# stulacy/bmm-mcmc

Measured on AMD Instinct MI355X. Metric: gibbs_sweeps_per_s, higher is better.
Workload: dtype f64; 1 GPU; c5: gibbs_collapsed K=20 N=10000000 P=100, 1 chain per GPU; sampler=collapsed, K=20, N=10000000, P=100, batch=2500000, chains=1, chains_per_gpu=1, burn_sweeps=30, x_layout=bit planes, ceil(P/32) words per observation, packed once at hand-over

## Files before the change

### bmm-mcmc_amd/csrc/chain.hip

```cpp
#include <hip/hip_runtime.h>
#include <hip/hip_ext.h>
#include <rccl/rccl.h>

#include <dlfcn.h>
#include <emmintrin.h>
#include <sched.h>
#include <sys/mman.h>

#include <cmath>
#include <cstdarg>
#include <cstdio>
#include <cstdint>
#include <cstdlib>
#include <cstring>
#include <atomic>
#include <chrono>
#include <condition_variable>
#include <exception>
#include <functional>
#include <limits>
#include <memory>
#include <mutex>
#include <new>
#include <string>
// ... 778 lines not shown
    if (old) HIP_TRY(hipStreamSynchronize(old));
    int rc = chain_stream_create(c, true);
    if (rc) { c->stream = old; c->stream_kind = old_kind; return rc; }
    chain_stream_release(c->device, old, old_kind);
    return BMM_OK;
}

struct Carver {
    char* base;
    size_t used = 0;
    template <class T> T* take(size_t n) {
        const size_t off = (used + 255) & ~(size_t)255;
        used = off + n * sizeof(T);
        return base ? reinterpret_cast<T*>(base + off) : nullptr;
    }
};

int chain_alloc(bmm_chain* c) {
    const ChainParams& p = c->p;
    HIP_TRY(hipSetDevice(c->device));
    {
        int rcs = chain_stream_create(c, false);
        if (rcs) return rcs;
    }
    const size_t nz = (size_t)p.N;
    const size_t ns = (size_t)p.K * p.P, nn = (size_t)p.K;
    const size_t ntab = (size_t)layout_of(c).doubles() + (explicit_params(p.mode) ? 0 : 2 * (size_t)pk_tq_doubles(layout_of(c)));
    auto carve = [&](Carver& a) {
        c->dNk = a.take<int32_t>(nn);
        c->dDNk = a.take<int32_t>(nn * kDeltaReps);
        c->dS = a.take<int32_t>(ns);
        c->dDS = a.take<int32_t>(ns * kDeltaReps);
        c->dTab = a.take<double>(ntab);
#ifdef BMM_DIAG
        c->dDiag = a.take<unsigned long long>(16);
#endif
        c->dSelfDone = a.take<int>(1);
        c->dViable = a.take<int>(1);
        c->dDNkAlt = a.take<int32_t>(nn * kDeltaReps);
        c->dDSAlt = a.take<int32_t>(ns * kDeltaReps);
#ifdef BMM_DEBUG_HOOKS
        c->dDbgFlag = a.take<int>(1);
        c->dPkStat = a.take<unsigned long long>(3);
#endif
        const size_t zeroed = a.used;
        c->dAlpha = a.take<double>(1);
        c->dPi = a.take<double>(nn);
        c->dTheta = a.take<double>(ns);
        c->dZ[0] = a.take<int32_t>(nz);
        c->dZ[1] = a.take<int32_t>(nz);
        return zeroed;
    };
    Carver measure{nullptr};
    carve(measure);
    c->arena = static_cast<char*>(dev_pool().get(c->device, measure.used, &c->arena_bytes));
    if (!c->arena) return set_err(BMM_E_HIP, "allocating the chain's state failed: %s", hipGetErrorString(hipGetLastError()));
    Carver real{c->arena};
    const size_t zeroed = carve(real);
    if (c->generic) HIP_TRY(hipMalloc(&c->dScratch, (size_t)c->scratch_stride * p.Kc * sizeof(double)));
    HIP_TRY(hipMemsetAsync(c->arena, 0, zeroed, c->stream));
    HIP_TRY(hipMemsetAsync(c->dZ[0], 0xff, nz * sizeof(int32_t), c->stream));
    HIP_TRY(hipMemcpyAsync(c->dAlpha, &c->alpha0, sizeof(double), hipMemcpyHostToDevice, c->stream));
    HIP_TRY(hipStreamSynchronize(c->stream));
    return BMM_OK;
}

int dbg_labels_ok(bmm_chain* c) {
#ifdef BMM_DEBUG_HOOKS
    int flag = 0;
    HIP_TRY(hipMemcpy(&flag, c->dDbgFlag, sizeof(int), hipMemcpyDeviceToHost));
    if (flag) return set_err(BMM_E_STATE, "a resample kernel produced or read a label outside [0, K): kernel bug (debug-hooks build check)");
#else
    (void)c;
#endif
    return BMM_OK;
}

int launch_resample(bmm_chain* c, const int32_t* z_in, int32_t* z_out, int64_t lo, int64_t hi,
                    uint32_t sweep) {
    ResampleArgs a{};
    a.X = c->dX; a.Xb = c->dXb; a.z_in = z_in; a.z_out = z_out; a.tab = c->dTab; a.dNk = c->dDNk; a.dS = c->dDS;
    a.lo = lo; a.hi = hi; a.sweep = sweep; a.minus_in_lds = c->minus_in_lds; a.diag = c->dDiag;
    a.dbg_flag = c->dDbgFlag; a.dbg_inject = (dbg_env("BMM_DEBUG_BADLABEL") ? 1 : 0) | (dbg_env("BMM_DEBUG_STRAGGLER") ? 2 : 0) |
                                             (dbg_env("BMM_DEBUG_DRAW_FALLBACK") ? 4 : 0) | (dbg_env("BMM_DEBUG_DRAW_NOEPS") ? 8 : 0);
    a.Nk = c->dNk; a.S = c->dS; a.alpha_ptr = c->dAlpha; a.self_done = c->dSelfDone;
#ifdef BMM_DEBUG_HOOKS
    a.pk_stat = c->dPkStat;
    a.pk_defer_every = c->pk_defer_every;
#endif
    const bool emit = c->probs_dst != nullptr;
    const bool use_generic = c->generic || (emit && !c->fn_emit);
    const bool self_launch = c->form.self && !emit && !use_generic;
    if (self_launch) { a.dNk_prev = c->dDNk; a.dS_prev = c->dDS; a.dNk = c->dDNkAlt; a.dS = c->dDSAlt; }
    const KernelForm& form = emit ? c->form_emit : c->form;
    const int gmax = emit ? c->grid_max_emit : c->grid_max;
    const int64_t ntiles = use_generic ? 1 : (hi - lo + tile_of(form) - 1) / tile_of(form);
    int grid = (int)(ntiles < gmax ? ntiles : gmax);
    if (use_generic) {
        const int64_t nt256 = (hi - lo + 255) / 256;
        const int64_t maxb = c->scratch_stride / 256;
        grid = (int)(nt256 < maxb ? nt256 : maxb);
    }
    if (emit) { a.wts = c->dWts; a.wtot = c->dWtot; }
    hipEvent_t e0 = nullptr, e1 = nullptr;
    if (c->prof > 0 && sweep % (uint32_t)c->prof == 0) {
        if (c->ev_used + 2 > c->ev.size()) {
            hipEvent_t a0, a1;
            HIP_TRY(hipEventCreate(&a0));
            HIP_TRY(hipEventCreate(&a1));
            c->ev.push_back(a0); c->ev.push_back(a1);
        }
        e0 = c->ev[c->ev_used]; e1 = c->ev[c->ev_used + 1];
        c->ev_used += 2;
    }
    if (use_generic) {
        if (e0) hipExtLaunchKernelGGL(k_resample_generic, dim3(grid), dim3(256), 0, c->stream, e0, e1, 0, c->p, a,
                                      c->dScratch, c->scratch_stride);
        else hipLaunchKernelGGL(k_resample_generic, dim3(grid), dim3(256), 0, c->stream, c->p, a, c->dScratch,
                                c->scratch_stride);
    } else {
        const resample_fn fn = emit ? c->fn_emit : c->fn;
        const int nt = form.nt;
        const size_t lds = emit ? c->lds_bytes_base : c->lds_bytes;
        if (e0) hipExtLaunchKernelGGL(fn, dim3(grid), dim3(nt), (uint32_t)lds, c->stream, e0, e1, 0, c->p, a);
        else hipLaunchKernelGGL(fn, dim3(grid), dim3(nt), lds, c->stream, c->p, a);
    }
    HIP_TRY(hipGetLastError());
    if (self_launch) { std::swap(c->dDNk, c->dDNkAlt); std::swap(c->dDS, c->dDSAlt); }
    if (emit) {
        const int64_t nb = (hi - lo + 255) / 256;
        hipLaunchKernelGGL(k_probs_finish, dim3((unsigned)(nb < 4096 ? nb : 4096)), dim3(256), 0, c->stream, c->p,
                           c->dTab, c->dWts, c->dWtot, z_in, lo, hi, c->probs_dst);
        HIP_TRY(hipGetLastError());
    }
    return BMM_OK;
}

int probs_alloc(bmm_chain* c, bool with_matrix) {
    const size_t n = (size_t)c->p.N;
    if (c->bits && !c->generic && !c->fn_emit) {
        const resample_fn fn = lookup(c->form_emit);
        int pe = 0;
        const hipError_t e = kernel_fits(fn, c->form_emit.nt, c->lds_bytes_base, &pe);
        if (e != hipSuccess) return set_err(BMM_E_HIP, "kernel set-up failed: %s", hipGetErrorString(e));
        c->fn_emit = fn;
        c->grid_max_emit = (pe < 1 ? 1 : pe) * c->num_cus;
    }
    if (!c->dWts) HIP_TRY(hipMalloc(&c->dWts, n * c->p.Kc * sizeof(double)));
    if (!c->dWtot) HIP_TRY(hipMalloc(&c->dWtot, n * sizeof(double)));
    if (with_matrix && !c->dProbs) HIP_TRY(hipMalloc(&c->dProbs, n * c->p.K * sizeof(double)));
    if (!c->fn_emit && !c->dScratch) {
        c->scratch_stride = generic_threads(c->p.Kc);
        HIP_TRY(hipMalloc(&c->dScratch, (size_t)c->scratch_stride * c->p.Kc * sizeof(double)));
    }
    return BMM_OK;
}

int launch_reduce_deltas(bmm_chain* c) {
    const int n = c->p.K * c->p.P + c->p.K;
    hipLaunchKernelGGL(k_reduce_deltas, dim3((n + 255) / 256), dim3(256), 0, c->stream, c->p, c->dDNk, c->dDS);
    HIP_TRY(hipGetLastError());
    return BMM_OK;
}

int launch_count_tables(bmm_chain* c) {
    if (c->alloc_on)
        hipLaunchKernelGGL(k_alloc_tables, dim3(c->p.KT), dim3(kCountTablesThreads), 0, c->stream, c->p, c->dNk, c->dS,
                           c->dDNk, c->dDS, (const int32_t*)c->dEaK, c->alloc_a, c->dTab);
    else if (c->temper_on)
        hipLaunchKernelGGL(k_temper_tables, dim3(c->p.KT), dim3(kCountTablesThreads), 0, c->stream, c->p, c->dNk, c->dS,
                           c->dDNk, c->dDS, (const double*)c->dAlpha, c->temper_b, c->dTab);
    else if (c->fs_mask)
        hipLaunchKernelGGL(k_count_tables<true>, dim3(c->p.KT), dim3(kCountTablesThreads), 0, c->stream, c->p, c->dNk, c->dS,
                           c->dDNk, c->dDS, c->dAlpha, c->dTab, (const uint32_t*)c->dFsMask, 0);
    else
        hipLaunchKernelGGL(k_count_tables<false>, dim3(c->p.KT), dim3(kCountTablesThreads), 0, c->stream, c->p, c->dNk, c->dS,
                           c->dDNk, c->dDS, c->dAlpha, c->dTab, (const uint32_t*)nullptr, c->form.pk && !c->generic ? 1 : 0);
    HIP_TRY(hipGetLastError());
    return BMM_OK;
}

int launch_score(bmm_chain* c, ScoreArgs a, bool loo) {
    const ChainParams& p = c->p;
    a.tab = c->dTab;
    if (!explicit_params(p.mode)) {
        double* const tab = loo ? c->dLooTab : c->dPredTab;
// ... 4344 lines not shown
                if (d == ch->slot) return set_err(BMM_E_ARG, "one chain per device here; chains on one device share (bmm_chain_share_data)");
            if (ch->p.N != chains[0]->p.N || ch->p.P != chains[0]->p.P) return set_err(BMM_E_ARG, "the chains differ in N or P");
            devs.push_back(ch->slot);
            int rc = bmm_chain_planes(ch, &bufs[(size_t)c], &words);
            if (rc) return rc;
        }
        int rc = rccl_broadcast_words(devs, bufs, (size_t)words);
        for (int c = 1; c < n_chains && rc == BMM_OK; ++c) rc = bmm_chain_planes_filled(chains[c]);
        return rc;
    });
}

int bmm_multi_selfcheck(int n_devices, const int* devices, int64_t words) {
    return guarded([&]() -> int {
        if (n_devices < 1 || !devices || words < 1) return set_err(BMM_E_ARG, "bad argument");
        std::vector<int> devs(devices, devices + n_devices);
        for (int q = 0; q < n_devices; ++q)
            for (int r2 = 0; r2 < q; ++r2)
                if (devs[(size_t)q] == devs[(size_t)r2]) return set_err(BMM_E_ARG, "devices must be distinct");
        std::vector<uint32_t> pat((size_t)words), got((size_t)words);
        for (int64_t i = 0; i < words; ++i) pat[(size_t)i] = (uint32_t)i * 2654435761u + 12345u;
        std::vector<DevBuf> bufs((size_t)n_devices);
        std::vector<void*> ptrs((size_t)n_devices);
        for (int q = 0; q < n_devices; ++q) {
            HIP_TRY(hipSetDevice(devs[(size_t)q]));
            HIP_TRY(bufs[(size_t)q].alloc((size_t)words * 4));
            ptrs[(size_t)q] = bufs[(size_t)q].p;
            if (q == 0) HIP_TRY(hipMemcpy(ptrs[0], pat.data(), (size_t)words * 4, hipMemcpyHostToDevice));
            else HIP_TRY(hipMemset(ptrs[(size_t)q], 0, (size_t)words * 4));
        }
        if (n_devices == 1) {
            Rccl r;
            int rc = rccl_open(r);
            if (rc) return rc;
            ncclComm_t comm = nullptr;
            ncclResult_t e = r.CommInitAll(&comm, 1, devs.data());
            if (e != ncclSuccess) return set_err(BMM_E_RCCL, "ncclCommInitAll failed: %s", r.GetErrorString(e));
            hipStream_t st = nullptr;
            hipError_t he = hipStreamCreateWithFlags(&st, hipStreamNonBlocking);
            if (he == hipSuccess) {
                e = r.Broadcast(ptrs[0], ptrs[0], (size_t)words, ncclUint32, 0, comm, st);
                he = hipStreamSynchronize(st);
                (void)hipStreamDestroy(st);
            }
            (void)r.CommDestroy(comm);
            if (he != hipSuccess) return set_err(BMM_E_HIP, "self-check stream failed: %s", hipGetErrorString(he));
            if (e != ncclSuccess) return set_err(BMM_E_RCCL, "ncclBroadcast failed: %s", r.GetErrorString(e));
        } else {
            int rc = rccl_broadcast_words(devs, ptrs, (size_t)words);
            if (rc) return rc;
        }
        for (int q = 0; q < n_devices; ++q) {
            HIP_TRY(hipSetDevice(devs[(size_t)q]));
            HIP_TRY(hipMemcpy(got.data(), ptrs[(size_t)q], (size_t)words * 4, hipMemcpyDeviceToHost));
            if (std::memcmp(got.data(), pat.data(), (size_t)words * 4) != 0)
                return set_err(BMM_E_RCCL, "device %d holds different words after the broadcast", devs[(size_t)q]);
        }
        return BMM_OK;
    });
}

int bmm_device_math(int device, int op, const double* in, const double* in2, double* out, int64_t n) {
    if (!in || !out || n < 0 || op < 0 || op > 5) return set_err(BMM_E_ARG, "bad argument");
    if (op == 2 && !in2) return set_err(BMM_E_ARG, "division needs in2");
    HIP_TRY(hipSetDevice(device));
    DevBuf bi, bi2, bo;
    HIP_TRY(bi.alloc(n * sizeof(double)));
    HIP_TRY(bo.alloc(n * sizeof(double)));
    HIP_TRY(hipMemcpy(bi.p, in, n * sizeof(double), hipMemcpyHostToDevice));
    if (in2) {
        HIP_TRY(bi2.alloc(n * sizeof(double)));
        HIP_TRY(hipMemcpy(bi2.p, in2, n * sizeof(double), hipMemcpyHostToDevice));
    }
    if (op == 5)
        hipLaunchKernelGGL(k_test_lgamma, dim3((unsigned)((n + 255) / 256)), dim3(256), 0, 0, bi.as<double>(), bo.as<double>(), n);
    else
        hipLaunchKernelGGL(k_test_math, dim3((unsigned)((n + 255) / 256)), dim3(256), 0, 0, op, bi.as<double>(),
                           bi2.as<double>(), bo.as<double>(), n);
    HIP_TRY(hipGetLastError());
    HIP_TRY(hipMemcpy(out, bo.p, n * sizeof(double), hipMemcpyDeviceToHost));
    return BMM_OK;
}

int bmm_device_variates(int device, int kind, double p, double q, uint64_t seed, uint32_t sweep, double* out,
                        int64_t n) {
    if (!out || n < 0 || kind < 0 || kind > 2) return set_err(BMM_E_ARG, "bad argument");
    HIP_TRY(hipSetDevice(device));
    DevBuf bo;
    HIP_TRY(bo.alloc(n * sizeof(double)));
    hipLaunchKernelGGL(k_test_variates, dim3((unsigned)((n + 255) / 256)), dim3(256), 0, 0, kind, p, q, seed, sweep,
                       bo.as<double>(), n);
    HIP_TRY(hipGetLastError());
    HIP_TRY(hipMemcpy(out, bo.p, n * sizeof(double), hipMemcpyDeviceToHost));
    return BMM_OK;
}

}
```

### bmm-mcmc_amd/csrc/kernels.hip.h

```cpp
#pragma once
#include <hip/hip_runtime.h>
#include <stdint.h>

#include "bmm_spec.h"

namespace bmm {

typedef __attribute__((address_space(3))) double lds_f64;

constexpr int kMaxP = 128;
constexpr int lcm_(int a, int b) { int x = a; while (x % b) x += a; return x; }
constexpr int kChunkP = kMaxP / lcm_(lcm_(kGroupW, kGroupWAlt), kGroupWm) * lcm_(lcm_(kGroupW, kGroupWAlt), kGroupWm);
constexpr int kMaxCats = 64;
constexpr int kMaxCatsAny = 1024;

enum : int { MODE_COLLAPSED = 0, MODE_DP = 1, MODE_SB = 2, MODE_FULL = 3 };
__host__ __device__ inline bool explicit_params(int mode) { return mode == MODE_SB || mode == MODE_FULL; }

struct TableLayout {
    int G, KT, Gm, M;
    __host__ __device__ int tp() const { return 0; }
    __host__ __device__ int cp() const { return G * KT * M; }
    __host__ __device__ int cm() const { return cp() + KT; }
    __host__ __device__ int nk() const { return cm() + KT; }
// ... 1044 lines not shown
typedef float pk_f2 __attribute__((ext_vector_type(2)));
typedef __attribute__((address_space(3))) pk_f2 lds_pk_f2;
typedef __attribute__((address_space(3))) float lds_f32;
constexpr int kOwnPadMax = ((kMaxP + kGroupWm - 1) / kGroupWm + kOwnSub - 1) / kOwnSub * kOwnSub;
static_assert(kOwnPadMax <= 64, "pk_exact_count loads the own-cluster entries one per lane");

__device__ __forceinline__ int pk_dp_label(const int32_t* NkT, int K, int Kused, int new_label, int zo, int zoc) {
    const int own_single = (zo >= 0 && NkT[zoc] == 1) ? 1 : 0;
    if (Kused - own_single < K - 1) {
        int zn = new_label;
        if (own_single && (zn < 0 || zo < zn)) zn = zo;
        return zn;
    }
    int best = -1, bs = 0;
    for (int k = 0; k < K; ++k) {
        const int sz = NkT[k] - (k == zo ? 1 : 0);
        if (sz > 0 && (best < 0 || sz < bs)) { best = k; bs = sz; }
    }
    return best >= 0 ? best : zoc;
}
__device__ __forceinline__ unsigned pk_field(int bit, unsigned mask, uint32_t b0, uint32_t b1, uint32_t b2, uint32_t b3) {
    const int wd = bit >> 5;
    return __builtin_amdgcn_alignbit(word_of(wd + 1, b0, b1, b2, b3), word_of(wd, b0, b1, b2, b3), (unsigned)(bit & 31)) & mask;
}

__device__ __forceinline__ double pk_bcast(double x, int j) {
    const long long b = __double_as_longlong(x);
    const uint64_t e = (uint64_t)(uint32_t)__builtin_amdgcn_readlane((int)(uint32_t)b, j) |
                       ((uint64_t)(uint32_t)__builtin_amdgcn_readlane((int)(uint32_t)(b >> 32), j) << 32);
    return __longlong_as_double((long long)e);
}

template <int KT, int GW>
__device__ __forceinline__ int pk_exact_count(const ChainParams& p, const ResampleArgs& a, const TableLayout& L,
                                              uint32_t w0, uint32_t w1, uint32_t w2, uint32_t w3, int zo, double u,
                                              const lds_f64* ET, int lane) {
    constexpr int GM = 1 << GW;
    constexpr int GR = KT <= 4 ? 6 : KT <= 8 ? 10 : 20;
    static_assert((kMaxP + GW - 1) / GW <= 64, "lane g holds the field of group g");
    const int G = p.G;
    const int zoc = zo < 0 ? 0 : zo;
    const int k = lane < KT ? lane : KT - 1;
    const double* const tp = a.tab + L.tp();
    const int gmp = L.gm_pad();
    const int go = lane < gmp ? lane : gmp - 1;
    const double oe = a.tab[L.tm() + ((size_t)go * KT + zoc) * kGroupMm + pk_field(go * kGroupWm, kGroupMm - 1, w0, w1, w2, w3)];
    const unsigned koff = (unsigned)k * GM;
    const int gl = lane < G ? lane : G - 1;
    const int fld = (int)pk_field(gl * GW, GM - 1, w0, w1, w2, w3);
    double sc = 0.0;
#pragma unroll 1
    for (int g0 = 0; g0 < G; g0 += GR) {
        double tv[GR];
#pragma unroll
        for (int v = 0; v < GR; ++v) {
            const int g = g0 + v < G ? g0 + v : G - 1;
            const double* const row = tp + ((size_t)g * KT * GM + (unsigned)__builtin_amdgcn_readlane(fld, g));
            tv[v] = row[koff];
        }
#pragma unroll
        for (int v = 0; v < GR; ++v)
            if (g0 + v < G) sc = sc + tv[v];
    }
    double own = 0.0;
#pragma unroll 1
    for (int g = 0; g < gmp; ++g) own = own + pk_bcast(oe, g);
    if (k == zo) sc = own;
    double m = neg_inf();
#pragma unroll
    for (int j = 0; j < KT; ++j) m = max_score(m, pk_bcast(sc, j));
    const double w = expw_tab(sc - m, ET);
    double run = 0.0, cdf = 0.0;
#pragma unroll
    for (int j = 0; j < KT; ++j) {
        run = run + pk_bcast(w, j);
        cdf = lane == j ? run : cdf;
    }
    const double t = u * run;
    int zn = (int)__popcll(__ballot(lane < KT && t >= cdf));
    if (!(m > neg_inf())) zn = zoc;
    return zn;
}

template <int KT, int NT, int GW>
__global__ __launch_bounds__(NT) void k_resample_pk(ChainParams p, ResampleArgs a) {
    static_assert(KT % 2 == 0 && KT <= 32, "pairs of categories, one lane per category in pk_exact_count");
    constexpr int GM = 1 << GW;
    constexpr int KP = KT / 2;
    constexpr int CH = KP <= 12 ? KP : KP / 2;
    static_assert(KP % CH == 0, "chunking");
    constexpr int NW = NT / 64;
    extern __shared__ __attribute__((aligned(16))) char smem[];
    const TableLayout L{p.G, KT, p.Gm, GM};
    double* const lds = reinterpret_cast<double*>(smem);
    const int nq_d = pk_tq_doubles(L), tail_d = L.tm() - L.nk();
    const volatile lds_pk_f2* const Tq = (const volatile lds_pk_f2*)lds;
    const volatile lds_f32* const Tm32 = (const volatile lds_f32*)(lds + nq_d);
    double* const tail = lds + 2 * nq_d;
    const int32_t* const NkT = reinterpret_cast<const int32_t*>(tail);
    const lds_f64* const ET = (const lds_f64*)(tail + (L.et() - L.nk()));
    int32_t* const hist = reinterpret_cast<int32_t*>(tail + tail_d);
    const int P = p.P, G = p.G, K = p.K;
    const int tid = threadIdx.x, lane = tid & 63;
    int* const next_chunk = hist + K * P + K;
    DIAG(const unsigned long long d_entry = diag_stamp();)
    const int64_t nchunks = (a.hi - a.lo + 63) / 64;
    const int64_t cpw = (nchunks + gridDim.x - 1) / gridDim.x;
    const int64_t wg_c0 = (int64_t)blockIdx.x * cpw;
    const int64_t wg_cn = nchunks - wg_c0 < cpw ? nchunks - wg_c0 : cpw;
    const int W = (P + 31) / 32;
    const int wave = __builtin_amdgcn_readfirstlane(tid >> 6);
    int64_t tile = wg_c0 + wave;
    const bool has_tile = wave < wg_cn;
    TilePos pos = tile_pos(a, has_tile ? tile : 0, 64, lane, lane);
    uint32_t b0 = 0, b1 = 0, b2 = 0, b3 = 0;
    if (has_tile) load_words(a.Xb, p.N, W, pos.ic, b0, b1, b2, b3);
    {
        auto stage = [&](const double* from, double* to, int n2) {
            const double2* src = reinterpret_cast<const double2*>(from);
            double2* dst = reinterpret_cast<double2*>(to);
            for (int i0 = tid; i0 < n2; i0 += NT * 8) {
                double2 t[8];
#pragma unroll
                for (int u = 0; u < 8; ++u) {
                    const int i = i0 + u * NT;
                    t[u] = src[i < n2 ? i : n2 - 1];
                }
#pragma unroll
                for (int u = 0; u < 8; ++u) {
                    const int i = i0 + u * NT;
                    if (i < n2) dst[i] = t[u];
                }
            }
        };
        stage(a.tab + L.doubles(), lds, nq_d);
        stage(a.tab + L.nk(), tail, tail_d / 2);
    }
    for (int i = tid; i < K * P + K; i += NT) hist[i] = 0;
    if (tid == 0) *next_chunk = NW;
    __syncthreads();
    DIAG(const unsigned long long d_staged = diag_stamp();)

    int Kused = 0, new_label = -1;
    if (p.mode == MODE_DP) {
        for (int k = 0; k < K; ++k) {
            if (NkT[k] > 0) ++Kused;
            else if (new_label < 0) new_label = k;
        }
    }
    float unit = kPkEpsUnit;
#ifdef BMM_DEBUG_HOOKS
    if (a.dbg_inject & 8) unit = 0.0f;
    unsigned ndeferred = 0, nunselected = 0;
#endif

    if (has_tile) {
        int zo = a.z_in ? a.z_in[pos.ic] : -1;
        asm volatile("" : "+v"(zo));
        int zn_prev = 0;
        int64_t i_prev = -1;
        for (;;) {
            const int zoc = zo < 0 ? 0 : zo;
            if (i_prev >= 0) a.z_out[i_prev] = zn_prev;
            int nc = 0;
            if (lane == 0) nc = atomicAdd(next_chunk, 1);
            nc = __builtin_amdgcn_readfirstlane(nc);
            const int64_t next = wg_c0 + nc;
            const bool has_next = nc < wg_cn;
            const TilePos npos = tile_pos(a, has_next ? next : tile, 64, lane, lane);
            uint32_t n0 = 0, n1 = 0, n2 = 0, n3 = 0;
            int zo_next = -1;

            pk_f2 acc[KP];
#pragma unroll
            for (int j = 0; j < KP; ++j) acc[j] = pk_f2{0.0f, 0.0f};
            float own32 = 0.0f;
            const volatile lds_f32* const orow0 = Tm32 + zoc * GM;
            __builtin_amdgcn_s_setprio(BMM_LOOKUP_PRIO);
#pragma unroll 1
            for (int h = 0; h < W; ++h) {
                if (has_next && h == 0) {
                    load_words(a.Xb, p.N, W, npos.ic, n0, n1, n2, n3);
                    if (a.z_in) zo_next = a.z_in[npos.ic];
                }
                const uint32_t cur = word_of(h, b0, b1, b2, b3), nxt = word_of(h + 1, b0, b1, b2, b3);
                const int g_lo = (32 * h + GW - 1) / GW;
                int g_hi = (32 * (h + 1) + GW - 1) / GW;
                g_hi = g_hi < G ? g_hi : G;
#pragma unroll 1
                for (int g = g_lo; g < g_hi; ++g) {
                    const unsigned nib = __builtin_amdgcn_alignbit(nxt, cur, (unsigned)(g * GW - 32 * h)) & (unsigned)(GM - 1);
                    const volatile lds_pk_f2* row = Tq + ((size_t)g * KP * GM + nib);
                    const volatile lds_f32* orow = orow0 + ((size_t)g * KT * GM + nib);
#pragma unroll
                    for (int c0 = 0; c0 < KP; c0 += CH) {
                        pk_f2 tv[CH];
                        float ov = 0.0f;
#pragma unroll
                        for (int j = 0; j < CH; ++j) tv[j] = row[(c0 + j) * GM];
                        if (c0 == 0) ov = *orow;
#pragma unroll
                        for (int j = 0; j < CH; ++j) acc[c0 + j] = acc[c0 + j] + tv[j];
                        if (c0 == 0) own32 = own32 + ov;
                        if (CH < KP) __builtin_amdgcn_sched_barrier(0);
                    }
                }
            }
            __builtin_amdgcn_s_setprio(0);
            float sc[KT];
            float m = -__builtin_inff();
#pragma unroll
            for (int k = 0; k < KT; ++k) {
                float v = (k & 1) ? acc[k >> 1].y : acc[k >> 1].x;
                if (k == zo) v = own32;
                sc[k] = v;
                m = __builtin_fmaxf(m, v);
            }
            const double u = z_uniform(p.seed, (uint64_t)(p.obs0 + pos.ic), a.sweep);
            int cnt = 0;
            bool certain = draw_pk<KT>(sc, m, u, G, unit, cnt);
            DBG_TIER1_FORCE(a, certain);
            bool defer = pos.valid && !certain;
#ifdef BMM_DEBUG_HOOKS
            const bool selected = a.pk_defer_every > 0 && pos.valid && pos.i % a.pk_defer_every == 0;
            nunselected += (unsigned)__popcll(__ballot(defer && !selected));
            defer = defer || selected;
#endif
            int zn = cnt;
            unsigned long long o = __ballot(defer);
#ifdef BMM_DEBUG_HOOKS
            ndeferred += (unsigned)__popcll(o);
#endif
            while (o) {
                const int src = __ffsll((long long)o) - 1;
                o &= o - 1;
                const uint32_t w0 = __builtin_amdgcn_readlane(b0, src), w1 = __builtin_amdgcn_readlane(b1, src);
                const uint32_t w2 = __builtin_amdgcn_readlane(b2, src), w3 = __builtin_amdgcn_readlane(b3, src);
                const int e = pk_exact_count<KT, GW>(p, a, L, w0, w1, w2, w3, __builtin_amdgcn_readlane(zo, src),
                                                     pk_bcast(u, src), ET, lane);
                if (lane == src) zn = e;
            }
            if (p.mode == MODE_DP && zn == K) zn = pk_dp_label(NkT, K, Kused, new_label, zo, zoc);
            const bool keep = pos.valid;
            BMM_DBG_LABELS(a, keep, pos.i == a.lo, K, zn, zo);
            count_movers(keep && zn >= 0 && zn != zo, zo, zn, b0, b1, b2, b3, hist, K, P, lane);
            zn_prev = zn;
            i_prev = keep ? pos.i : -1;
            if (!has_next) break;
            b0 = n0; b1 = n1; b2 = n2; b3 = n3;
            zo = zo_next;
            pos = npos;
            tile = next;
        }
        if (i_prev >= 0) a.z_out[i_prev] = zn_prev;
    }

    DIAG(const unsigned long long d_loop = diag_stamp();)
    __syncthreads();
    DIAG(const unsigned long long d_sync = diag_stamp();)
    flush_hist(hist, K, P, a.dS + (size_t)(blockIdx.x % kDeltaReps) * K * P, a.dNk + (blockIdx.x % kDeltaReps) * K, tid, NT);
    DIAG(asm volatile("s_waitcnt vmcnt(0)" ::: "memory"); const unsigned long long d_flush = diag_stamp();)
    DIAG(if (a.diag && tid == 0) {
        atomicAdd(&a.diag[5], 1ull); atomicAdd(&a.diag[7], 1ull); atomicAdd(&a.diag[14], d_flush - d_entry);
        atomicAdd(&a.diag[8], d_staged - d_entry); atomicAdd(&a.diag[9], d_loop - d_staged);
        atomicAdd(&a.diag[10], d_sync - d_loop); atomicAdd(&a.diag[11], d_flush - d_sync);
    })
#ifdef BMM_DEBUG_HOOKS
    if (a.pk_stat) {
        if (tid == 0) {
            int64_t first = a.lo + wg_c0 * 64, last = a.lo + (wg_c0 + (wg_cn > 0 ? wg_cn : 0)) * 64;
            last = last < a.hi ? last : a.hi;
            if (last > first) atomicAdd(&a.pk_stat[0], (unsigned long long)(last - first));
        }
        if (lane == 0 && ndeferred) atomicAdd(&a.pk_stat[1], (unsigned long long)ndeferred);
        if (lane == 0 && nunselected) atomicAdd(&a.pk_stat[2], (unsigned long long)nunselected);
    }
#endif
}

__device__ __forceinline__ unsigned field_from_x(const int32_t* X, const uint32_t* Xb, int64_t N, int P,
                                                  int64_t i, int g, int GW) {
    if (Xb) {
        const int o = g * GW, w = o >> 5, sh = o & 31, W = (P + 31) >> 5;
        uint32_t v = Xb[(int64_t)w * N + i] >> sh;
        if (sh + GW > 32 && w + 1 < W) v |= Xb[(int64_t)(w + 1) * N + i] << (32 - sh);
        return v & (unsigned)((1 << GW) - 1);
    }
    unsigned nib = 0;
    for (int j = 0; j < GW; ++j) {
        const int d = g * GW + j;
        if (d < P) nib |= ((unsigned)X[i + (int64_t)d * N] & 1u) << j;
    }
    return nib;
}

__global__ __launch_bounds__(256) void k_resample_generic(ChainParams p, ResampleArgs a, double* scr,
                                                          int64_t stride) {
    const bool has_minus = !explicit_params(p.mode);
    const TableLayout L = layout_of(p, has_minus);
    const int GM = L.M;
    const double* const Tp = a.tab + L.tp();
    const double* const Tm = a.tab + L.tm();
    const int32_t* const NkT = reinterpret_cast<const int32_t*>(a.tab + L.nk());
    const double* const ET = a.tab + L.et();
    const int P = p.P, G = p.G, K = p.K, Kc = p.Kc, KT = p.KT;
    const int64_t gid = (int64_t)blockIdx.x * blockDim.x + threadIdx.x;
    double* const my = scr + gid;

    int Kused = 0, new_label = -1;
    if (p.mode == MODE_DP) {
        for (int k = 0; k < K; ++k) {
            if (NkT[k] > 0) ++Kused;
            else if (new_label < 0) new_label = k;
        }
    }
    for (int64_t i = a.lo + gid; i < a.hi; i += (int64_t)gridDim.x * blockDim.x) {
        int zo = a.z_in ? a.z_in[i] : -1;
        const int zoc = zo < 0 ? 0 : zo;
        double acc_own = 0.0;
        if (has_minus)
            for (int g = 0; g < p.Gm; ++g)
                acc_own = acc_own + Tm[((size_t)g * KT + zoc) * kGroupMm + field_from_x(a.X, a.Xb, p.N, P, i, g, kGroupWm)];
        double m = neg_inf();
        for (int k0 = 0; k0 < Kc; k0 += 16) {
            double acc[16];
#pragma unroll
            for (int j = 0; j < 16; ++j) acc[j] = 0.0;
            for (int g = 0; g < G; ++g) {
                const double* row = Tp + ((size_t)g * KT + k0) * GM + field_from_x(a.X, a.Xb, p.N, P, i, g, p.W);
#pragma unroll
                for (int j = 0; j < 16; ++j)
                    if (k0 + j < Kc) acc[j] = acc[j] + row[j * GM];
            }
#pragma unroll
            for (int j = 0; j < 16; ++j) {
                const int k = k0 + j;
                if (k < Kc) {
                    double sc = acc[j];
                    if (has_minus && k == zo) sc = acc_own;
                    my[(int64_t)k * stride] = sc;
                    m = __builtin_fmax(m, sc);
                }
            }
        }
        double run = 0.0;
        for (int k = 0; k < Kc; ++k) {
            const double w = expw_tab(my[(int64_t)k * stride] - m, ET);
            if (a.wts) a.wts[(int64_t)k * p.N + i] = w;
            run = run + w;
            my[(int64_t)k * stride] = run;
        }
        const double tot = run;
        if (a.wts) a.wtot[i] = tot;
// ... 651 lines not shown
            if (!LOO) my[(int64_t)k * stride] = w;
        }
        if (has_minus) tot = tot + expw_tab(ownv - mx, ET);
        const double ld = seated ? mx + log_(tot) : qnan();
        if (a.out) a.out[i] = ld;
        if (LOO) {
            if (a.acc) loo_fold(a, i, ld, ET);
            continue;
        }
        if (a.run_max) predict_fold(a, i, ld, ET);
        if (a.resp || a.resp_acc)
            for (int k = 0; k < Kc; ++k) {
                const double r = div_(my[(int64_t)k * stride], tot);
                if (a.resp) a.resp[(int64_t)k * a.rows + i] = r;
                if (a.resp_acc) a.resp_acc[(int64_t)k * a.rows + i] += r;
            }
    }
}

__global__ __launch_bounds__(256) void k_loo_reset(int64_t N, double* __restrict__ acc) {
    for (int64_t i = (int64_t)blockIdx.x * 256 + threadIdx.x; i < N; i += (int64_t)gridDim.x * 256) {
        acc[LOO_MAX * N + i] = neg_inf();
        acc[LOO_SUM * N + i] = 0.0;
        acc[LOO_MIN * N + i] = pos_inf();
        acc[LOO_S1 * N + i] = 0.0;
        acc[LOO_S2 * N + i] = 0.0;
        acc[LOO_MEAN * N + i] = 0.0;
        acc[LOO_M2 * N + i] = 0.0;
    }
}

__global__ __launch_bounds__(256) void k_loo_finish(int64_t N, int n, const double* __restrict__ acc,
                                                    double* __restrict__ out) {
    const double ln = log_((double)n);
    for (int64_t i = (int64_t)blockIdx.x * 256 + threadIdx.x; i < N; i += (int64_t)gridDim.x * 256) {
        const double s1 = acc[LOO_S1 * N + i];
        out[0 * N + i] = (ln + acc[LOO_MIN * N + i]) - log_(s1);
        out[1 * N + i] = div_(s1 * s1, acc[LOO_S2 * N + i]);
        out[2 * N + i] = (acc[LOO_MAX * N + i] + log_(acc[LOO_SUM * N + i])) - ln;
        out[3 * N + i] = acc[LOO_MEAN * N + i];
        out[4 * N + i] = n > 1 ? div_(acc[LOO_M2 * N + i], (double)(n - 1)) : qnan();
    }
}

__global__ __launch_bounds__(1024) void k_loo_reduce(int64_t N, const double* __restrict__ out, double* __restrict__ scal) {
    __shared__ double sh[4][1024];
    const int t = threadIdx.x;
    double cpo = 0.0, lp = 0.0, vr = 0.0, es = pos_inf();
    for (int64_t i = t; i < N; i += 1024) {
        cpo = cpo + out[0 * N + i];
        es = __builtin_fmin(es, out[1 * N + i]);
        lp = lp + out[2 * N + i];
        vr = vr + out[4 * N + i];
    }
    sh[0][t] = cpo; sh[1][t] = es; sh[2][t] = lp; sh[3][t] = vr;
    __syncthreads();
    for (int s = 512; s > 0; s >>= 1) {
        if (t < s) {
            sh[0][t] = sh[0][t] + sh[0][t + s];
            sh[1][t] = __builtin_fmin(sh[1][t], sh[1][t + s]);
            sh[2][t] = sh[2][t] + sh[2][t + s];
            sh[3][t] = sh[3][t] + sh[3][t + s];
        }
        __syncthreads();
    }
    if (t == 0) {
        scal[0] = sh[0][0]; scal[1] = sh[1][0]; scal[2] = sh[2][0]; scal[3] = sh[3][0];
        scal[4] = sh[2][0] - sh[3][0];
    }
}

__global__ void k_test_math(int op, const double* in, const double* in2, double* out, int64_t n) {
    const int64_t i = (int64_t)blockIdx.x * blockDim.x + threadIdx.x;
    if (i >= n) return;
    const double x = in[i];
    double y;
    if (op == 0) y = log_(x);
    else if (op == 1) y = exp_(x);
    else if (op == 2) y = div_(x, in2[i]);
    else if (op == 3) y = sqrt_(x);
    else y = expw_(x);
    out[i] = y;
}
__global__ void k_test_variates(int kind, double pp, double qq, uint64_t seed, uint32_t sweep, double* out,
                                int64_t n) {
    const int64_t i = (int64_t)blockIdx.x * blockDim.x + threadIdx.x;
    if (i >= n) return;
    double y;
    if (kind == 0) {
        Stream s = make_stream(seed, (uint32_t)i, sweep, kStreamThetaA);
        y = rgamma_(pp, s);
    } else if (kind == 1) {
        Stream sa = make_stream(seed, (uint32_t)i, sweep, kStreamThetaA);
        Stream sb = make_stream(seed, (uint32_t)i, sweep, kStreamThetaB);
        y = rbeta_(pp, qq, sa, sb);
    } else {
        y = update_alpha_(pp, 1.0, 1.0, 1000.0, (int)qq, seed + (uint64_t)i, sweep);
    }
    out[i] = y;
}

constexpr int kPtThreads = 256;
constexpr int kPtMaxLdsK = 64;

template <class T>
__device__ inline T pt_block_sum(T v, T* slot) {
    const int tid = threadIdx.x;
    __syncthreads();
    slot[tid] = v;
    __syncthreads();
    for (int h = kPtThreads / 2; h > 0; h >>= 1) {
        if (tid < h) slot[tid] += slot[tid + h];
        __syncthreads();
    }
    return slot[0];
}
__device__ inline double pt_f(uint32_t n) { return n ? (double)n * log_((double)n) : 0.0; }

template <class L>
__global__ __launch_bounds__(256) void k_pt_narrow(const int32_t* __restrict__ src, int64_t ss, int64_t si, int base,
                                                   int S, int64_t i0, int64_t rows, int Kc, L* __restrict__ out,
                                                   int64_t pitch, int* __restrict__ flag) {
    __shared__ int32_t tile[32][33];
    const int64_t b0 = (int64_t)blockIdx.x * 32;
    const int s0 = blockIdx.y * 32;
    const int tx = threadIdx.x & 31, ty = threadIdx.x >> 5;
    for (int r = ty; r < 32; r += 8) {
        if (si == 1) {
            const int s = s0 + r;
            const int64_t li = b0 + tx;
            tile[r][tx] = (s < S && li < rows) ? src[(size_t)s * ss + li] : base;
        } else {
            const int s = s0 + tx;
            const int64_t li = b0 + r;
            tile[tx][r] = (s < S && li < rows) ? src[(size_t)s * ss + (size_t)li * si] : base;
        }
    }
    __syncthreads();
    for (int r = ty; r < 32; r += 8) {
        const int s = s0 + r;
        const int64_t li = b0 + tx;
        if (s < S && li < rows) {
            int v = tile[r][tx] - base;
            if ((uint32_t)v >= (uint32_t)Kc) { *flag = 1; v = 0; }
            out[(size_t)s * pitch + i0 + li] = (L)v;
        }
    }
}

template <class L>
__global__ __launch_bounds__(256) void k_pt_sizes(const L* __restrict__ lab, int64_t pitch, int64_t N, int Kc,
                                                  uint64_t* __restrict__ A, double* __restrict__ F) {
    extern __shared__ uint32_t pt_lds[];
    __shared__ uint64_t su[kPtThreads];
    __shared__ double sd[kPtThreads];
    const int tid = threadIdx.x;
    for (int k = tid; k < 4 * Kc; k += kPtThreads) pt_lds[k] = 0;
    __syncthreads();
    const L* __restrict__ row = lab + (size_t)blockIdx.x * pitch;
    uint32_t* const h = pt_lds + (tid >> 6) * Kc;
    for (int64_t i = tid; i < N; i += kPtThreads) atomicAdd(&h[(uint32_t)row[i]], 1u);
    __syncthreads();
    uint64_t a = 0;
    double f = 0.0;
    for (int k = tid; k < Kc; k += kPtThreads) {
        const uint32_t n = pt_lds[k] + pt_lds[Kc + k] + pt_lds[2 * Kc + k] + pt_lds[3 * Kc + k];
// ... 1379 lines not shown
```

Baseline: 3406 sweeps/s.

## Trim register pressure in packed resample kernel via 32-bit offsets and lazy kernarg reads

The packed resample kernel now uses 32-bit chunk offsets with host-rebased pointers, so 64-bit index arithmetic drops out of the hot loop. Rarely used values (ChainParams/ResampleArgs fields, LDS table pointers, the DP label scan) are reloaded from the kernarg segment only inside unlikely branches, which frees scalar and vector registers for the common path. The draw is rewritten over packed float pairs, and when observation indices fit in 32 bits the Philox key is computed once per wave. A debug test kernel checks that the new draw matches the old one. The risks are reliance on the kernarg layout, and RNG-key or bookkeeping mismatches if the rebasing or the key shortcut is wrong.

```diff
diff --git a/bmm-mcmc_amd/csrc/chain.hip b/bmm-mcmc_amd/csrc/chain.hip
--- a/bmm-mcmc_amd/csrc/chain.hip
+++ b/bmm-mcmc_amd/csrc/chain.hip
@@ -884,7 +884,8 @@
     a.X = c->dX; a.Xb = c->dXb; a.z_in = z_in; a.z_out = z_out; a.tab = c->dTab; a.dNk = c->dDNk; a.dS = c->dDS;
     a.lo = lo; a.hi = hi; a.sweep = sweep; a.minus_in_lds = c->minus_in_lds; a.diag = c->dDiag;
     a.dbg_flag = c->dDbgFlag; a.dbg_inject = (dbg_env("BMM_DEBUG_BADLABEL") ? 1 : 0) | (dbg_env("BMM_DEBUG_STRAGGLER") ? 2 : 0) |
-                                             (dbg_env("BMM_DEBUG_DRAW_FALLBACK") ? 4 : 0) | (dbg_env("BMM_DEBUG_DRAW_NOEPS") ? 8 : 0);
+                                             (dbg_env("BMM_DEBUG_DRAW_FALLBACK") ? 4 : 0) | (dbg_env("BMM_DEBUG_DRAW_NOEPS") ? 8 : 0) |
+                                             (dbg_env("BMM_DEBUG_PK_GENKEY") ? 16 : 0);
     a.Nk = c->dNk; a.S = c->dS; a.alpha_ptr = c->dAlpha; a.self_done = c->dSelfDone;
 #ifdef BMM_DEBUG_HOOKS
     a.pk_stat = c->dPkStat;
@@ -904,6 +905,11 @@
         grid = (int)(nt256 < maxb ? nt256 : maxb);
     }
     if (emit) { a.wts = c->dWts; a.wtot = c->dWtot; }
+    if (form.pk && !use_generic) {
+        a.Xb += lo;
+        if (a.z_in) a.z_in += lo;
+        a.z_out += lo;
+    }
     hipEvent_t e0 = nullptr, e1 = nullptr;
     if (c->prof > 0 && sweep % (uint32_t)c->prof == 0) {
         if (c->ev_used + 2 > c->ev.size()) {
@@ -5414,6 +5420,33 @@
     return BMM_OK;
 }
 
+#ifdef BMM_DEBUG_HOOKS
+int bmm_dbg_pk_draw(int device, int kt, int spec, const float* scores, const double* u, int G, int64_t n, int* out) {
+    if (!scores || !u || !out || n < 0) return set_err(BMM_E_ARG, "bad argument");
+    if (kt != 4 && kt != 12 && kt != 20 && kt != 32)
+        return set_err(BMM_E_ARG, "the draw is instantiated for 4, 12, 20 and 32 accumulators");
+    HIP_TRY(hipSetDevice(device));
+    DevBuf bs, bu, bo;
+    HIP_TRY(bs.alloc((size_t)n * kt * sizeof(float)));
+    HIP_TRY(bu.alloc((size_t)n * sizeof(double)));
+    HIP_TRY(bo.alloc((size_t)n * 2 * sizeof(int)));
+    HIP_TRY(hipMemcpy(bs.p, scores, (size_t)n * kt * sizeof(float), hipMemcpyHostToDevice));
+    HIP_TRY(hipMemcpy(bu.p, u, (size_t)n * sizeof(double), hipMemcpyHostToDevice));
+    const dim3 grid((unsigned)((n + 255) / 256));
+#define BMM_TEST_PK_DRAW(KT)                                                                                              \
+    if (spec) hipLaunchKernelGGL((k_test_pk_draw<KT, true>), grid, dim3(256), 0, 0, bs.as<float>(), bu.as<double>(), G, n, bo.as<int>()); \
+    else hipLaunchKernelGGL((k_test_pk_draw<KT, false>), grid, dim3(256), 0, 0, bs.as<float>(), bu.as<double>(), G, n, bo.as<int>())
+    if (kt == 4) { BMM_TEST_PK_DRAW(4); }
+    else if (kt == 12) { BMM_TEST_PK_DRAW(12); }
+    else if (kt == 20) { BMM_TEST_PK_DRAW(20); }
+    else { BMM_TEST_PK_DRAW(32); }
+#undef BMM_TEST_PK_DRAW
+    HIP_TRY(hipGetLastError());
+    HIP_TRY(hipMemcpy(out, bo.p, (size_t)n * 2 * sizeof(int), hipMemcpyDeviceToHost));
+    return BMM_OK;
+}
+#endif
+
 int bmm_device_variates(int device, int kind, double p, double q, uint64_t seed, uint32_t sweep, double* out,
                         int64_t n) {
     if (!out || n < 0 || kind < 0 || kind > 2) return set_err(BMM_E_ARG, "bad argument");
diff --git a/bmm-mcmc_amd/csrc/kernels.hip.h b/bmm-mcmc_amd/csrc/kernels.hip.h
--- a/bmm-mcmc_amd/csrc/kernels.hip.h
+++ b/bmm-mcmc_amd/csrc/kernels.hip.h
@@ -1150,6 +1150,107 @@
     return zn;
 }
 
+struct PkArgsView {
+    const ChainParams* p;
+    const ResampleArgs* a;
+};
+static_assert(alignof(ChainParams) == 8 && alignof(ResampleArgs) == 8 && sizeof(ChainParams) % 8 == 0,
+              "k_resample_pk(ChainParams, ResampleArgs): the second argument lies right behind the first");
+__device__ __forceinline__ PkArgsView pk_args_view() {
+    const __attribute__((address_space(4))) char* ka =
+        (const __attribute__((address_space(4))) char*)__builtin_amdgcn_kernarg_segment_ptr();
+    asm volatile("" : "+s"(ka));
+    PkArgsView v;
+    v.p = (const ChainParams*)ka;
+    v.a = (const ResampleArgs*)(ka + sizeof(ChainParams));
+    return v;
+}
+struct PkLds {
+    const int32_t* NkT;
+    const lds_f64* ET;
+    int32_t* hist;
+};
+__device__ __forceinline__ PkLds pk_lds(char* smem, const TableLayout& L) {
+    double* const tail = reinterpret_cast<double*>(smem) + 2 * pk_tq_doubles(L);
+    PkLds r;
+    r.NkT = reinterpret_cast<const int32_t*>(tail);
+    r.ET = (const lds_f64*)(tail + (L.et() - L.nk()));
+    r.hist = reinterpret_cast<int32_t*>(tail + (L.tm() - L.nk()));
+    return r;
+}
+
+struct PkPos {
+    uint32_t s0;
+    uint32_t loff;
+    bool valid;
+};
+__device__ __forceinline__ PkPos pk_pos(uint32_t n, int chunk, int lane) {
+    PkPos t;
+    t.s0 = (uint32_t)chunk << 6;
+    const uint32_t room = n - 1u - t.s0;
+    t.valid = (uint32_t)lane <= room;
+    t.loff = (uint32_t)lane < room ? (uint32_t)lane : room;
+    return t;
+}
+template <class T>
+__device__ __forceinline__ T* pk_at(T* sbase, uint32_t loff) {
+    static_assert(sizeof(T) == 4, "words and labels");
+    return (T*)((const char*)sbase + (loff * 4u));
+}
+__device__ __forceinline__ void pk_load_words(const uint32_t* Xb, int64_t N, int W, const PkPos& t, uint32_t& w0,
+                                              uint32_t& w1, uint32_t& w2, uint32_t& w3) {
+    const uint32_t* const b = Xb + t.s0;
+    w0 = *pk_at(b, t.loff);
+    if (W > 1) w1 = *pk_at(b + N, t.loff);
+    if (W > 2) w2 = *pk_at(b + 2 * N, t.loff);
+    if (W > 3) w3 = *pk_at(b + 3 * N, t.loff);
+}
+
+template <int KT>
+__device__ __forceinline__ bool pk_draw2(const pk_f2 (&s2)[KT / 2], float m, double u, int G, float unit, int& cnt) {
+    static_assert(KT % 2 == 0 && KT <= kTier1MaxCats, "the band is derived for at most kTier1MaxCats categories");
+    constexpr int KP = KT / 2;
+    const pk_f2 mm{m, m}, l2e{0x1.715476p+0f, 0x1.715476p+0f};
+    pk_f2 c[KP];
+    float run = 0.0f;
+#pragma unroll
+    for (int j = 0; j < KP; ++j) {
+        const pk_f2 x = (s2[j] - mm) * l2e;
+        run = run + __builtin_amdgcn_exp2f(x.x);
+        c[j].x = run;
+        run = run + __builtin_amdgcn_exp2f(x.y);
+        c[j].y = run;
+    }
+    const float t = (float)u * run;
+    const pk_f2 tt{t, t};
+    float nearest = __builtin_inff();
+    int n = 0;
+#pragma unroll
+    for (int j = 0; j < KP; ++j) {
+        const pk_f2 diff = tt - c[j];
+        n += diff.x >= 0.0f ? 1 : 0;
+        nearest = __builtin_fminf(nearest, __builtin_fabsf(diff.x));
+        n += diff.y >= 0.0f ? 1 : 0;
+        nearest = __builtin_fminf(nearest, __builtin_fabsf(diff.y));
+    }
+    cnt = n;
+    return nearest > pk_band(m, G, unit) * run && m > -__builtin_inff() && m < __builtin_inff();
+}
+__device__ __forceinline__ double pk_uniform(uint64_t seed, uint64_t i0, uint32_t s0, uint32_t loff, uint32_t sweep,
+                                             bool key_uniform) {
+    uint32_t ra, rb;
+    if (key_uniform) {
+        uint32_t k = z_key(seed, 0);
+        asm volatile("" : "+s"(k));
+        philox2x32_10((uint32_t)i0 + s0 + loff, sweep, k, ra, rb);
+        asm volatile("" : "+v"(ra), "+v"(rb));
+    } else {
+        const uint64_t i = i0 + s0 + loff;
+        philox2x32_10((uint32_t)i, sweep, z_key(seed, i), ra, rb);
+    }
+    return u52(ra, rb);
+}
+
 template <int KT, int NT, int GW>
 __global__ __launch_bounds__(NT) void k_resample_pk(ChainParams p, ResampleArgs a) {
     static_assert(KT % 2 == 0 && KT <= 32, "pairs of categories, one lane per category in pk_exact_count");
@@ -1165,24 +1266,22 @@
     const volatile lds_pk_f2* const Tq = (const volatile lds_pk_f2*)lds;
     const volatile lds_f32* const Tm32 = (const volatile lds_f32*)(lds + nq_d);
     double* const tail = lds + 2 * nq_d;
-    const int32_t* const NkT = reinterpret_cast<const int32_t*>(tail);
-    const lds_f64* const ET = (const lds_f64*)(tail + (L.et() - L.nk()));
     int32_t* const hist = reinterpret_cast<int32_t*>(tail + tail_d);
     const int P = p.P, G = p.G, K = p.K;
     const int tid = threadIdx.x, lane = tid & 63;
     int* const next_chunk = hist + K * P + K;
     DIAG(const unsigned long long d_entry = diag_stamp();)
-    const int64_t nchunks = (a.hi - a.lo + 63) / 64;
-    const int64_t cpw = (nchunks + gridDim.x - 1) / gridDim.x;
-    const int64_t wg_c0 = (int64_t)blockIdx.x * cpw;
-    const int64_t wg_cn = nchunks - wg_c0 < cpw ? nchunks - wg_c0 : cpw;
+    const uint32_t n = (uint32_t)(a.hi - a.lo);
+    const int nchunks = (int)((n + 63u) >> 6);
+    const int cpw = (nchunks + (int)gridDim.x - 1) / (int)gridDim.x;
+    const int wg_c0 = (int)blockIdx.x * cpw;
+    const int wg_cn = nchunks - wg_c0 < cpw ? nchunks - wg_c0 : cpw;
     const int W = (P + 31) / 32;
     const int wave = __builtin_amdgcn_readfirstlane(tid >> 6);
-    int64_t tile = wg_c0 + wave;
     const bool has_tile = wave < wg_cn;
-    TilePos pos = tile_pos(a, has_tile ? tile : 0, 64, lane, lane);
+    PkPos pos = pk_pos(n, has_tile ? wg_c0 + wave : 0, lane);
     uint32_t b0 = 0, b1 = 0, b2 = 0, b3 = 0;
-    if (has_tile) load_words(a.Xb, p.N, W, pos.ic, b0, b1, b2, b3);
+    if (has_tile) pk_load_words(a.Xb, p.N, W, pos, b0, b1, b2, b3);
     {
         auto stage = [&](const double* from, double* to, int n2) {
             const double2* src = reinterpret_cast<const double2*>(from);
@@ -1209,13 +1308,6 @@
     __syncthreads();
     DIAG(const unsigned long long d_staged = diag_stamp();)
 
-    int Kused = 0, new_label = -1;
-    if (p.mode == MODE_DP) {
-        for (int k = 0; k < K; ++k) {
-            if (NkT[k] > 0) ++Kused;
-            else if (new_label < 0) new_label = k;
-        }
-    }
     float unit = kPkEpsUnit;
 #ifdef BMM_DEBUG_HOOKS
     if (a.dbg_inject & 8) unit = 0.0f;
@@ -1223,21 +1315,37 @@
 #endif
 
     if (has_tile) {
-        int zo = a.z_in ? a.z_in[pos.ic] : -1;
+        const uint32_t* const Xb = a.Xb;
+        const int32_t* const z_in = a.z_in;
+        int32_t* const z_out = a.z_out;
+        const int64_t N = p.N;
+        const uint64_t seed = p.seed, i0 = (uint64_t)(p.obs0 + a.lo);
+        const uint32_t sweep = a.sweep;
+        int key_general = (int)(uint32_t)(((uint64_t)(p.obs0 + a.hi) - 1u) >> 32);
+#ifdef BMM_DEBUG_HOOKS
+        if (a.dbg_inject & 16) key_general = 1;
+#endif
+        key_general = __builtin_amdgcn_readfirstlane(key_general);
+        const int dp_K = p.mode == MODE_DP ? K : -1;
+        const int has_zin = (int)((uint32_t)((uintptr_t)z_in >> 32) | (uint32_t)(uintptr_t)z_in);
+        int zo = -1;
+        if (z_in) zo = *pk_at(z_in + pos.s0, pos.loff);
         asm volatile("" : "+v"(zo));
         int zn_prev = 0;
-        int64_t i_prev = -1;
+        uint32_t st_s0 = 0, st_loff = 0;
+        bool st_on = false;
         for (;;) {
             const int zoc = zo < 0 ? 0 : zo;
-            if (i_prev >= 0) a.z_out[i_prev] = zn_prev;
+            if (st_on) *pk_at(z_out + st_s0, st_loff) = zn_prev;
             int nc = 0;
             if (lane == 0) nc = atomicAdd(next_chunk, 1);
             nc = __builtin_amdgcn_readfirstlane(nc);
-            const int64_t next = wg_c0 + nc;
             const bool has_next = nc < wg_cn;
-            const TilePos npos = tile_pos(a, has_next ? next : tile, 64, lane, lane);
+            const PkPos npos = pk_pos(n, has_next ? wg_c0 + nc : 0, lane);
             uint32_t n0 = 0, n1 = 0, n2 = 0, n3 = 0;
             int zo_next = -1;
+            int Wl = W, zl = has_zin;
+            asm volatile("" : "+s"(Wl), "+s"(zl));
 
             pk_f2 acc[KP];
 #pragma unroll
@@ -1248,8 +1356,8 @@
 #pragma unroll 1
             for (int h = 0; h < W; ++h) {
                 if (has_next && h == 0) {
-                    load_words(a.Xb, p.N, W, npos.ic, n0, n1, n2, n3);
-                    if (a.z_in) zo_next = a.z_in[npos.ic];
+                    pk_load_words(Xb, N, Wl, npos, n0, n1, n2, n3);
+                    if (zl) zo_next = *pk_at(z_in + npos.s0, npos.loff);
                 }
                 const uint32_t cur = word_of(h, b0, b1, b2, b3), nxt = word_of(h + 1, b0, b1, b2, b3);
                 const int g_lo = (32 * h + GW - 1) / GW;
@@ -1275,22 +1383,27 @@
                 }
             }
             __builtin_amdgcn_s_setprio(0);
-            float sc[KT];
+            pk_f2 s2[KP];
             float m = -__builtin_inff();
 #pragma unroll
-            for (int k = 0; k < KT; ++k) {
-                float v = (k & 1) ? acc[k >> 1].y : acc[k >> 1].x;
-                if (k == zo) v = own32;
-                sc[k] = v;
-                m = __builtin_fmaxf(m, v);
-            }
-            const double u = z_uniform(p.seed, (uint64_t)(p.obs0 + pos.ic), a.sweep);
+            for (int j = 0; j < KP; ++j) {
+                float x = acc[j].x, y = acc[j].y;
+                if (2 * j == zo) x = own32;
+                if (2 * j + 1 == zo) y = own32;
+                s2[j] = pk_f2{x, y};
+                m = __builtin_fmaxf(m, x);
+                m = __builtin_fmaxf(m, y);
+            }
+            int kg = key_general;
+            asm volatile("" : "+s"(kg));
+            const double u = pk_uniform(seed, i0, pos.s0, pos.loff, sweep, kg == 0);
             int cnt = 0;
-            bool certain = draw_pk<KT>(sc, m, u, G, unit, cnt);
+            bool certain = pk_draw2<KT>(s2, m, u, G, unit, cnt);
             DBG_TIER1_FORCE(a, certain);
             bool defer = pos.valid && !certain;
 #ifdef BMM_DEBUG_HOOKS
-            const bool selected = a.pk_defer_every > 0 && pos.valid && pos.i % a.pk_defer_every == 0;
+            const bool selected = a.pk_defer_every > 0 && pos.valid &&
+                                  (a.lo + (int64_t)pos.s0 + lane) % a.pk_defer_every == 0;
             nunselected += (unsigned)__popcll(__ballot(defer && !selected));
             defer = defer || selected;
 #endif
@@ -1299,34 +1412,67 @@
 #ifdef BMM_DEBUG_HOOKS
             ndeferred += (unsigned)__popcll(o);
 #endif
-            while (o) {
-                const int src = __ffsll((long long)o) - 1;
-                o &= o - 1;
-                const uint32_t w0 = __builtin_amdgcn_readlane(b0, src), w1 = __builtin_amdgcn_readlane(b1, src);
-                const uint32_t w2 = __builtin_amdgcn_readlane(b2, src), w3 = __builtin_amdgcn_readlane(b3, src);
-                const int e = pk_exact_count<KT, GW>(p, a, L, w0, w1, w2, w3, __builtin_amdgcn_readlane(zo, src),
-                                                     pk_bcast(u, src), ET, lane);
-                if (lane == src) zn = e;
-            }
-            if (p.mode == MODE_DP && zn == K) zn = pk_dp_label(NkT, K, Kused, new_label, zo, zoc);
+            if (__builtin_expect(o != 0, 0)) {
+                const PkArgsView v = pk_args_view();
+                const TableLayout Lc{v.p->G, KT, v.p->Gm, GM};
+                const PkLds lc = pk_lds(smem, Lc);
+                int ln = lane;
+                asm volatile("" : "+v"(ln));
+                do {
+                    const int src = __ffsll((long long)o) - 1;
+                    o &= o - 1;
+                    const uint32_t w0 = __builtin_amdgcn_readlane(b0, src), w1 = __builtin_amdgcn_readlane(b1, src);
+                    const uint32_t w2 = __builtin_amdgcn_readlane(b2, src), w3 = __builtin_amdgcn_readlane(b3, src);
+                    const int e = pk_exact_count<KT, GW>(*v.p, *v.a, Lc, w0, w1, w2, w3, __builtin_amdgcn_readlane(zo, src),
+                                                         pk_bcast(u, src), lc.ET, ln);
+                    if (ln == src) zn = e;
+                } while (o);
+            }
+            if (__builtin_expect(__ballot(zn == dp_K) != 0, 0)) {
+                const PkArgsView v = pk_args_view();
+                const int Kc = v.p->K;
+                const TableLayout Lc{v.p->G, KT, v.p->Gm, GM};
+                const int32_t* const Nkc = pk_lds(smem, Lc).NkT;
+                int Kused = 0, new_label = -1;
+                for (int k = 0; k < Kc; ++k) {
+                    if (Nkc[k] > 0) ++Kused;
+                    else if (new_label < 0) new_label = k;
+                }
+                if (zn == Kc) zn = pk_dp_label(Nkc, Kc, Kused, new_label, zo, zoc);
+            }
             const bool keep = pos.valid;
-            BMM_DBG_LABELS(a, keep, pos.i == a.lo, K, zn, zo);
-            count_movers(keep && zn >= 0 && zn != zo, zo, zn, b0, b1, b2, b3, hist, K, P, lane);
+#ifdef BMM_DEBUG_HOOKS
+            BMM_DBG_LABELS(a, keep, pos.s0 + (uint32_t)lane == 0u, K, zn, zo);
+#endif
+            const bool moves = keep && zn >= 0 && zn != zo;
+            if (__builtin_expect(__ballot(moves) != 0, 0)) {
+                const PkArgsView v = pk_args_view();
+                const int Kc = v.p->K, Pc = v.p->P;
+                const TableLayout Lc{v.p->G, KT, v.p->Gm, GM};
+                int ln = lane;
+                asm volatile("" : "+v"(ln));
+                count_movers(moves, zo, zn, b0, b1, b2, b3, pk_lds(smem, Lc).hist, Kc, Pc, ln);
+            }
             zn_prev = zn;
-            i_prev = keep ? pos.i : -1;
+            st_s0 = pos.s0; st_loff = pos.loff; st_on = keep;
             if (!has_next) break;
             b0 = n0; b1 = n1; b2 = n2; b3 = n3;
             zo = zo_next;
             pos = npos;
-            tile = next;
-        }
-        if (i_prev >= 0) a.z_out[i_prev] = zn_prev;
+        }
+        if (st_on) *pk_at(z_out + st_s0, st_loff) = zn_prev;
     }
 
     DIAG(const unsigned long long d_loop = diag_stamp();)
     __syncthreads();
     DIAG(const unsigned long long d_sync = diag_stamp();)
-    flush_hist(hist, K, P, a.dS + (size_t)(blockIdx.x % kDeltaReps) * K * P, a.dNk + (blockIdx.x % kDeltaReps) * K, tid, NT);
+    {
+        const PkArgsView v = pk_args_view();
+        const int Kc = v.p->K, Pc = v.p->P;
+        const TableLayout Lc{v.p->G, KT, v.p->Gm, GM};
+        const int rep = blockIdx.x % kDeltaReps;
+        flush_hist(pk_lds(smem, Lc).hist, Kc, Pc, v.a->dS + (size_t)rep * Kc * Pc, v.a->dNk + rep * Kc, tid, NT);
+    }
     DIAG(asm volatile("s_waitcnt vmcnt(0)" ::: "memory"); const unsigned long long d_flush = diag_stamp();)
     DIAG(if (a.diag && tid == 0) {
         atomicAdd(&a.diag[5], 1ull); atomicAdd(&a.diag[7], 1ull); atomicAdd(&a.diag[14], d_flush - d_entry);
@@ -1336,7 +1482,7 @@
 #ifdef BMM_DEBUG_HOOKS
     if (a.pk_stat) {
         if (tid == 0) {
-            int64_t first = a.lo + wg_c0 * 64, last = a.lo + (wg_c0 + (wg_cn > 0 ? wg_cn : 0)) * 64;
+            int64_t first = a.lo + (int64_t)wg_c0 * 64, last = a.lo + ((int64_t)wg_c0 + (wg_cn > 0 ? wg_cn : 0)) * 64;
             last = last < a.hi ? last : a.hi;
             if (last > first) atomicAdd(&a.pk_stat[0], (unsigned long long)(last - first));
         }
@@ -2154,6 +2300,32 @@
     else y = expw_(x);
     out[i] = y;
 }
+#ifdef BMM_DEBUG_HOOKS
+template <int KT, bool SPEC>
+__global__ __launch_bounds__(256) void k_test_pk_draw(const float* __restrict__ scores, const double* __restrict__ u,
+                                                      int G, int64_t n, int* __restrict__ out) {
+    const int64_t i = (int64_t)blockIdx.x * blockDim.x + threadIdx.x;
+    if (i >= n) return;
+    float sc[KT];
+    float m = -__builtin_inff();
+#pragma unroll
+    for (int k = 0; k < KT; ++k) {
+        sc[k] = scores[i * KT + k];
+        m = __builtin_fmaxf(m, sc[k]);
+    }
+    int cnt = 0;
+    bool ok;
+    if constexpr (SPEC) {
+        ok = draw_pk<KT>(sc, m, u[i], G, kPkEpsUnit, cnt);
+    } else {
+        pk_f2 s2[KT / 2];
+#pragma unroll
+        for (int j = 0; j < KT / 2; ++j) s2[j] = pk_f2{sc[2 * j], sc[2 * j + 1]};
+        ok = pk_draw2<KT>(s2, m, u[i], G, kPkEpsUnit, cnt);
+    }
+    out[2 * i] = cnt; out[2 * i + 1] = ok ? 1 : 0;
+}
+#endif
 __global__ void k_test_variates(int kind, double pp, double qq, uint64_t seed, uint32_t sweep, double* out,
                                 int64_t n) {
     const int64_t i = (int64_t)blockIdx.x * blockDim.x + threadIdx.x;
```

New measurement: 3565 sweeps/s (median of 6 runs). 1.05x the previous value.
